# phylo42/RAPPAS

Hardware: AMD Instinct MI355X
Metric: reads placed/sec (whole node), 150 bp DNA vs 10^7-kmer DB (higher is better)
Workload: dtype f32; 1 GPU; C2: DNA k=10, 999 branches, phylo-kmer DB of 786432 keys / 9995042 entries (seed 42), replicated per GPU; 10000000 x 150 symbol reads per GPU per step (uniform, seed 1+rank), keep_at_most=7; reads_per_gpu=10000000

## Files before the change

rappas_amd/csrc/rk_kernels.hip:

```cpp
#include "rk_device.h"
#include "rk_slots24.h"

#include <type_traits>
#ifndef RK_ROW_NT
#define RK_ROW_NT 0
#endif
#ifndef RK_ROW_AUX
#define RK_ROW_AUX 0
#endif
#ifndef RK_HEADS_MAX_K
#define RK_HEADS_MAX_K 16
#endif
#ifndef RK_ABLATE
#define RK_ABLATE 0
#endif
#include "../../include/rappas_place.h"

namespace rk {

#ifdef RK_STAMPS
__device__ unsigned long long rk_stamp_buf[2 * 4096 * 16];
__device__ __forceinline__ unsigned long long rk_now() {
    unsigned long long t;
    __builtin_amdgcn_sched_barrier(0);
    asm volatile("s_memtime %0\n\ts_waitcnt lgkmcnt(0)" : "=s"(t)::"memory");
    __builtin_amdgcn_sched_barrier(0);
    return t;
}
#define RK_STAMP(slot) do { unsigned long long n_ = rk_now(); st_[slot] += n_ - t_; t_ = n_; } while (0)
#define RK_STAMP_PARAMS , unsigned long long *st_, unsigned long long &t_
#define RK_STAMP_ARGS , st_, t_
#else
#define RK_STAMP(slot) do {} while (0)
#define RK_STAMP_PARAMS
#define RK_STAMP_ARGS
#endif

__device__ __forceinline__ u32 ord_f32(float f) {
    u32 u = __float_as_uint(f);
    return (u & 0x80000000u) ? ~u : (u | 0x80000000u);
}
__device__ __forceinline__ float unord_f32(u32 o) {
    u32 u = (o & 0x80000000u) ? (o & 0x7FFFFFFFu) : ~o;
    return __uint_as_float(u);
}
__device__ __forceinline__ u64 make_key(u32 raw_score_bits, u32 branch) {
    return ((u64)ord_f32(__uint_as_float(raw_score_bits)) << 32) | (u64)(0xFFFFu - branch);
}
__device__ __forceinline__ u64 shfl64(u64 v, int src, int width) {
    u32 lo = (u32)v, hi = (u32)(v >> 32);
    lo = __shfl(lo, src, width);
    hi = __shfl(hi, src, width);
    return ((u64)hi << 32) | lo;
}
__device__ __forceinline__ u64 shfl_xor64(u64 v, int m, int width) {
    u32 lo = (u32)v, hi = (u32)(v >> 32);
    lo = __shfl_xor(lo, m, width);
    hi = __shfl_xor(hi, m, width);
    return ((u64)hi << 32) | lo;
}
__device__ __forceinline__ double shfl_f64(double v, int src, int width) {
    return __longlong_as_double((long long)shfl64((u64)__double_as_longlong(v), src, width));
}
__device__ __forceinline__ bool tile_order_given(const PlaceArgs &a) { return a.perm != nullptr && *a.keep_order == 0u; }
__device__ __forceinline__ u32 batch_class(const PlaceArgs &a) { return a.keep_order[0] == 0u ? 2u : (a.keep_order[3] != 0u ? 1u : 0u); }
__device__ __forceinline__ bool batch_is_mine(const PlaceArgs &a) {
    if (!a.only_if || !a.perm) return true;
    return ((a.only_if >> batch_class(a)) & 1u) != 0u;
// ... 203 lines not shown
    c.cur = need ? off : c.cur;
    if (SOA) c.scur = need ? (off_t)(off + 2 * (off_t)len) : c.scur;
    const bool ok = lii < c.rem;
    if (SOA) {
        const off_t bo = ok ? (off_t)(c.cur + 2 * li) : (off_t)0;
        const off_t so = ok ? (off_t)(c.scur + 4 * li) : (off_t)0;
        br = *(const unsigned short *)(rows + bo);
        sc = *(const float *)(rows + so);
        c.cur += 2 * G;
        c.scur += 4 * G;
    } else {
        off_t eo = ok ? (off_t)(c.cur + 8 * li) : (off_t)0;
        if (RK_ABLATE & 16) eo = 0;
        const uint2 e = *(const uint2 *)(rows + eo);
        br = e.x;
        sc = __uint_as_float(e.y);
        c.cur += 8 * G;
    }
    c.rem -= G;
}

__device__ __forceinline__ void apply_entry(u32 *S, u32 nb, u32 br, float sc, float QT, float T, u32 br_base = 0) {
    if (RK_ABLATE & 8) {
        asm volatile("" ::"v"(br), "v"(sc));
        return;
    }
    const u32 idx = (br != 0xFFFFu) ? br - br_base : nb;
    const u32 old = S[idx];
    const float base = (old == S_UNTOUCHED) ? QT : __uint_as_float(old);
    const float d = sc - T;
    const float nw = base + d;
    S[idx] = __float_as_uint(nw);
}
template <bool MONO>
__device__ __forceinline__ float touch_base(u32 old, float QT) {
    float base;
    if (MONO) asm("v_max_f32 %0, %1, %2" : "=v"(base) : "v"(old), "v"(QT));
    else base = (old == S_UNTOUCHED) ? QT : __uint_as_float(old);
    return base;
}
template <bool MONO = false>
__device__ __forceinline__ void apply_delta(u32 *p, float d, float QT) {
    if (RK_ABLATE & 8) {
        asm volatile("" ::"v"(p), "v"(d));
        return;
    }
    *p = __float_as_uint(touch_base<MONO>(*p, QT) + d);
}
template <bool MONO = false>
__device__ __forceinline__ void apply_slot(u32 *S, u32 sb, float sc, float QT, float T) {
    apply_delta<MONO>((u32 *)((unsigned char *)S + sb), sc - T, QT);
}
template <int G, int U, bool WIDE, bool SOA = false>
__device__ __forceinline__ void accumulate_list(u32 *S, u32 nb, const u64 *list, int cnt, u32 li,
                                                const unsigned char *rows, float QT, float T, u32 s_lo = 0, u32 s_win = 0xFFFFu,
                                                u32 wlo4p4 = 4u, u32 w4 = 0xFFFFFFFFu) {
    Cursor<WIDE> c;
    c.h = -1; c.rem = 0; c.cur = 0; c.scur = 0;
    c.dn = list[0];
    u32 br[U];
    float sc[U];
#pragma unroll
    for (int u = 0; u < U; u++) cursor_issue<G, WIDE, SOA>(c, list, cnt, li, (int)li, rows, br[u], sc[u], s_lo, s_win);
    const bool win = !SOA && w4 != 0xFFFFFFFFu;
    auto slot_of = [&](u32 b) {
        if (SOA) {
            const u32 xw = b - s_lo;
            return (xw < s_win) ? (xw + 1u) * 4u : 0u;
        }
        const u32 t = b - wlo4p4;
        return win ? ((t < w4) ? t + 4u : 0u) : b;
    };
    while (true) {
#pragma unroll
        for (int u = 0; u < U; u++) {
            apply_slot(S, slot_of(br[u]), sc[u], QT, T);
            cursor_issue<G, WIDE, SOA>(c, list, cnt, li, (int)li, rows, br[u], sc[u], s_lo, s_win);
        }
        if (!__any(c.h < cnt)) break;
    }
#pragma unroll
    for (int u = 0; u < U; u++) apply_slot(S, slot_of(br[u]), sc[u], QT, T);
}

// ... 29 lines not shown

template <int G, int U, bool WIDE>
__device__ __forceinline__ void accumulate_chunks(u32 *S, u32 nb, const typename ItemT<WIDE>::type *items, int cnt,
                                                  u32 li, const unsigned char *rows, float QT, float T) {
    typedef typename ItemT<WIDE>::type item_t;
    const u32 li8 = li * 8;
    u32 br[U];
    float sc[U];
    item_t it[U];
#pragma unroll
    for (int u = 0; u < U; u++) chunk_issue<G, WIDE>(items[u], u < cnt, li, li8, rows, br[u], sc[u]);
#pragma unroll
    for (int u = 0; u < U; u++) it[u] = items[U + u];
    int s0 = 0;
    while (true) {
#pragma unroll
        for (int u = 0; u < U; u++) {
            apply_slot(S, br[u], sc[u], QT, T);
            chunk_issue<G, WIDE>(it[u], s0 + U + u < cnt, li, li8, rows, br[u], sc[u]);
            it[u] = items[s0 + 2 * U + u];
        }
        s0 += U;
        if (!__any(s0 < cnt)) break;
    }
}

constexpr u32 ITEM_FILLER = 0xFFFFFF00u;
typedef u32 v2u32 __attribute__((ext_vector_type(2)));

__device__ __forceinline__ __amdgpu_buffer_rsrc_t rows_resource(const DbView &db) {
    return __builtin_amdgcn_make_buffer_rsrc((void *)db.rows, (short)0, (int)(u32)db.rows_bytes, 0x00020000);
}

template <int G, int U, bool MONO, bool WIN = false, bool D24 = false>
__device__ __forceinline__ void accumulate_units(u32 *S, const u32 *items, int wcnt, u32 li,
                                                 __amdgpu_buffer_rsrc_t rs, float QT, float T, u32 wlo4p4 = 4u, u32 w4 = 0xFFFFFFFFu) {
    static_assert(!D24 || (G == 16 && !WIN), "dense units: 16-lane groups, whole trees");
    static_assert(rk_slots24::SLOT_BITS == SLOT24_BITS, "rk_slots24.h unpacks the slot words rk_device.h defines");
    const u32 li8 = li * 8;
    const u32 my_unit = li >> 4;
    const rk_slots24::Shifts sh24 = rk_slots24::lane_shifts(li);
    u32 sb[U], it[U];
    float sc[U];
    auto issue = [&](u32 item, u32 &b, float &v) {
        u32 off = item + li8;
        if (G > 16) off = (my_unit <= (item & 7u)) ? (item & ~127u) + li8 : ITEM_FILLER;
        if (RK_ABLATE & 16) off = li8;
        const v2u32 e = __builtin_amdgcn_raw_buffer_load_b64(rs, (int)off, 0, RK_ROW_AUX);
        b = e.x;
        v = __uint_as_float(e.y);
    };
    auto slot_of = [&](u32 b) {
        if (!WIN) return b;
        const u32 t = b - wlo4p4;
        return (t < w4) ? t + 4u : 0u;
    };
    auto prepare = [&](float v, u32 *&pa, u32 *&pb) {
        const int w = (int)__float_as_uint(v);
        const u32 r = (u32)__builtin_amdgcn_update_dpp(w, w, 0x128, 0xF, 0x3, false);
        const rk_slots24::Slots s = rk_slots24::lane_slots(sh24, r);
        pa = S + s.a;
        pb = S + s.b;
    };
#pragma unroll
    for (int u = 0; u < U; u++) issue(items[u], sb[u], sc[u]);
#pragma unroll
    for (int u = 0; u < U; u++) it[u] = items[U + u];
    int s0 = 0;
    if (D24) {
        u32 *pa, *pb;
        prepare(sc[0], pa, pb);
        while (true) {
#pragma unroll
            for (int u = 0; u < U; u++) {
                u32 *na, *nb;
                if (RK_ABLATE & 8) {
                    asm volatile("" ::"v"(pa), "v"(pb), "v"(sb[u]), "v"(sc[u]));
                    prepare(sc[(u + 1) % U], na, nb);
                } else {
                    const u32 oa = *pa, ob = *pb;
                    prepare(sc[(u + 1) % U], na, nb);
                    *pa = __float_as_uint(touch_base<MONO>(oa, QT) + __uint_as_float(sb[u]));
                    *pb = __float_as_uint(touch_base<MONO>(ob, QT) + sc[u]);
                }
                issue(it[u], sb[u], sc[u]);
                it[u] = items[s0 + 2 * U + u];
                pa = na;
                pb = nb;
            }
            s0 += U;
            if (s0 >= wcnt) break;
        }
        return;
    }
    while (true) {
#pragma unroll
        for (int u = 0; u < U; u++) {
            apply_slot<MONO>(S, slot_of(sb[u]), sc[u], QT, T);
            issue(it[u], sb[u], sc[u]);
            it[u] = items[s0 + 2 * U + u];
        }
        s0 += U;
        if (s0 >= wcnt) break;
    }
}

template <int S>
__device__ __forceinline__ u32 row_ror32(u32 v) {
    return (u32)__builtin_amdgcn_update_dpp(0, (int)v, 0x120 + S, 0xF, 0xF, false);
}
template <int G, int S>
__device__ __forceinline__ u64 group_rotate(u64 v, u32 li) {
    if (G == 16) {
        return ((u64)row_ror32<S>((u32)(v >> 32)) << 32) | row_ror32<S>((u32)v);
    } else {
        return shfl64(v, (int)((li + G - S) % G), G);
    }
}
template <int G, int S>
struct RankAbove {
    static __device__ __forceinline__ int run(u64 v, u32 li) {
        return ((group_rotate<G, S>(v, li) > v) ? 1 : 0) + RankAbove<G, S - 1>::run(v, li);
    }
};
template <int G>
struct RankAbove<G, 0> {
    static __device__ __forceinline__ int run(u64, u32) { return 0; }
};
template <int G>
__device__ __forceinline__ u64 group_max(u64 v) {
    if (G == 16) {
        u64 o;
        o = ((u64)row_ror32<8>((u32)(v >> 32)) << 32) | row_ror32<8>((u32)v); v = o > v ? o : v;
        o = ((u64)row_ror32<4>((u32)(v >> 32)) << 32) | row_ror32<4>((u32)v); v = o > v ? o : v;
        o = ((u64)row_ror32<2>((u32)(v >> 32)) << 32) | row_ror32<2>((u32)v); v = o > v ? o : v;
        o = ((u64)row_ror32<1>((u32)(v >> 32)) << 32) | row_ror32<1>((u32)v); v = o > v ? o : v;
        return v;
    } else {
#pragma unroll
        for (int s = 1; s < G; s <<= 1) {
            u64 o = shfl_xor64(v, s, G);
            v = o > v ? o : v;
        }
        return v;
    }
}

template <int G>
__device__ __forceinline__ int rank_candidates(const u64 *list, int c, u64 *win, int K, u32 li) {
    if (c <= G) {
        const u64 mine = ((int)li < c) ? list[li] : 0ull;
        const int rank = RankAbove<G, G - 1>::run(mine, li);
        if (mine != 0 && rank < K) win[rank] = mine;
    } else {
        for (int j = (int)li; j < c; j += G) {
            const u64 mine = list[j];
            int rank = 0;
            for (int t = 0; t < c; t++) rank += (list[t] > mine) ? 1 : 0;
            if (rank < K) win[rank] = mine;
        }
    }
    wave_lds_fence();
    return c < K ? c : K;
}

template <int G>
__device__ __forceinline__ int select_topk_scan(u32 *S, u32 ns, u32 li, u32 gi, int K, u64 *list, int cap, u64 &win_key RK_STAMP_PARAMS) {
    const u32 nb = ns;
    u64 *win = list + (cap - 16);
    const int capc = cap - 16;
    const uint4 *S4 = (const uint4 *)S;
    uint4 *S4w = (uint4 *)S;
    const u32 n4 = (nb + 3) / 4;
    float mo = -INFINITY;
    u32 mi = 0xFFFFFFFFu;
    for (u32 q = li; q < n4; q += G) {
        const uint4 v4 = S4[q];
        const u32 i = 4 * q;
        const float v[4] = {__uint_as_float(v4.x), __uint_as_float(v4.y), __uint_as_float(v4.z), __uint_as_float(v4.w)};
#pragma unroll
        for (int e = 0; e < 4; e++) {
            const bool gt = (v[e] > mo) && (i + e < nb);
            mo = gt ? v[e] : mo;
            mi = gt ? i + e : mi;
        }
    }
    const u64 km = (mi != 0xFFFFFFFFu) ? make_key(__float_as_uint(mo), mi - 1u) : 0ull;
    const int rank = RankAbove<G, G - 1>::run(km, li);
    u64 tau = group_max<G>((rank == K - 1) ? km : 0ull);
    int c = 0;
    const uint4 reset4 = make_uint4(S_UNTOUCHED, S_UNTOUCHED, S_UNTOUCHED, S_UNTOUCHED);
    for (u32 q0 = 0; q0 < n4; q0 += G) {
        const u32 q = q0 + li;
        uint4 v4 = reset4;
        if (q < n4) { v4 = S4[q]; S4w[q] = reset4; }
        const u32 i = 4 * q;
        const u32 raw[4] = {v4.x, v4.y, v4.z, v4.w};
        u64 key[4];
        bool any = false;
#pragma unroll
        for (int e = 0; e < 4; e++) {
            key[e] = (raw[e] != S_UNTOUCHED && i + e < nb) ? make_key(raw[e], i + e - 1u) : 0ull;
            any = any || (key[e] != 0 && key[e] >= tau);
        }
        if (group_bits<G>(__ballot(any), gi) == 0) continue;
#pragma unroll
        for (int e = 0; e < 4; e++) {
            const bool cand = key[e] != 0 && key[e] >= tau;
            const u64 sub = group_bits<G>(__ballot(cand), gi);
            if (sub == 0) continue;
            if (c + G > capc) {
                wave_lds_fence();
                const int kept = rank_candidates<G>(list, c, win, K, li);
                if ((int)li < kept) list[li] = win[li];
                if (kept == K) tau = win[K - 1];
                wave_lds_fence();
                c = kept;
            }
            const bool still = cand && key[e] >= tau;
            const u64 sub2 = group_bits<G>(__ballot(still), gi);
            if (still) list[c + count_below<G>(sub2, li)] = key[e];
            c += __builtin_popcountll(sub2);
        }
    }
    wave_lds_fence();
    const int num = rank_candidates<G>(list, c, win, K, li);
    win_key = ((int)li < num) ? win[li] : 0ull;
// ... 186 lines not shown
    const u32 n4_full = ns / 4;
    if (li < n4_full) {
        uint4 a = S4[li];
        u32 q = li + G;
        for (; q + G < n4_full; q += 2 * G) {
            const uint4 b = S4[q];
            heads3_feed_quad(h, a);
            a = S4[q + G];
            heads3_feed_quad(h, b);
        }
        if (q < n4_full) {
            const uint4 b = S4[q];
            heads3_feed_quad(h, a);
            a = b;
        }
        heads3_feed_quad(h, a);
    }
    if ((ns & 3u) && (n4_full % G) == li) {
        uint4 v4 = S4[n4_full];
        const u32 i = 4 * n4_full;
        if (i >= ns) v4.x = S_UNTOUCHED;
        if (i + 1 >= ns) v4.y = S_UNTOUCHED;
        if (i + 2 >= ns) v4.z = S_UNTOUCHED;
        if (i + 3 >= ns) v4.w = S_UNTOUCHED;
        heads3_feed_quad(h, v4);
    }
}
template <int S>
__device__ __forceinline__ u32 row_shr32(u32 v) {
    return (u32)__builtin_amdgcn_update_dpp(0, (int)v, 0x110 + S, 0xF, 0xF, true);
}
constexpr u32 HEADS3_SECOND = 128u;
template <int G>
__device__ __forceinline__ int heads3_rounds(const Heads3 &h, int K, u32 li, u32 gi, u32 &win_o, u32 &win_t, bool &doubt) {
    static_assert(4 * G < (int)HEADS3_SECOND, "stream tags");
    constexpr u32 ORD_NEG_INF = 0x007FFFFFu;
    u32 o0[4], o1[4], t0[4];
#pragma unroll
    for (int c = 0; c < 4; c++) {
        o0[c] = ord_f32(h.s0[c]); o1[c] = ord_f32(h.s1[c]);
        t0[c] = 4u * li + (u32)c + 1u;
    }
    u32 last = ORD_NEG_INF;
    int num = 0;
    win_o = 0; win_t = 0;
    for (int r = 0; r < K; r++) {
        const u32 m = group_max_u32<G>(max(max(o0[0], o0[1]), max(o0[2], o0[3])));
        const bool valid = m != ORD_NEG_INF;
        u32 cand = 0;
#pragma unroll
        for (int c = 0; c < 4; c++) cand = max(cand, (o0[c] == m) ? t0[c] : 0u);
        const u32 w = group_max_u32<G>(valid ? cand : 0u);
        const bool mine = (int)li == r && valid;
        win_o = mine ? m : win_o;
        win_t = mine ? w : win_t;
        num += valid ? 1 : 0;
        last = valid ? m : last;
#pragma unroll
        for (int c = 0; c < 4; c++) {
            const bool pop = valid && t0[c] == w;
            o0[c] = pop ? o1[c] : o0[c];
            o1[c] = pop ? ORD_NEG_INF : o1[c];
            t0[c] = pop ? (t0[c] | HEADS3_SECOND) : t0[c];
        }
    }
    u32 od = max(max(ord_f32(h.dr[0]), ord_f32(h.dr[1])), max(ord_f32(h.dr[2]), ord_f32(h.dr[3])));
    od = max(od, max(max(o0[0], o0[1]), max(o0[2], o0[3])));
    const bool d = (num == K) ? (od >= last) : (od != ORD_NEG_INF);
    doubt = group_bits<G>(__ballot(d), gi) != 0;
    return num;
}
template <int G>
__device__ __forceinline__ u32 heads3_locate(const u32 *S, u32 ns, u32 stream, u32 bits, bool second) {
    constexpr u32 NONE = 0x40000000u;
    constexpr int CH = 8;
    const u32 n4 = (ns + 3) / 4;
    const int trip = (int)((n4 + G - 1) / G);
    const int cnt = (int)((ns - stream + 4u * G - 1u) / (4u * G));
    int k = (trip - 1) / CH;
    const u32 *p = S + stream + (u32)(4 * G * CH) * (u32)k;
    u32 first = NONE, sec = NONE;
    {
        const int jv = cnt - CH * k;
        u32 w[CH];
#pragma unroll
        for (int j = 0; j < CH; j++) {
            const u32 *pj = (j < jv) ? p + 4 * G * j : S;
            w[j] = *pj;
        }
#pragma unroll
        for (int j = CH - 1; j >= 0; j--) {
            const bool eq = w[j] == bits;
            sec = eq ? first : sec;
            first = eq ? (u32)j : first;
        }
    }
    for (k--; k >= 0; k--) {
        p -= 4 * G * CH;
        first += (u32)CH; sec += (u32)CH;
        u32 w[CH];
#pragma unroll
        for (int j = 0; j < CH; j++) w[j] = p[4 * G * j];
#pragma unroll
        for (int j = CH - 1; j >= 0; j--) {
            const bool eq = w[j] == bits;
            sec = eq ? first : sec;
            first = eq ? (u32)j : first;
        }
    }
    const u32 i = second ? sec : first;
    return i < NONE ? stream + 4u * G * i : 0u;
}
template <int G>
__device__ __forceinline__ int heads3_select(u32 *S, u32 ns, u32 li, u32 gi, int K, u64 *list, int cap, u64 &win_key, bool &doubt RK_STAMP_PARAMS) {
    Heads3 h;
    heads3_clear(h);
    heads3_scan<G>(S, ns, li, h);
    RK_STAMP(8);
    u32 win_o, win_t;
    const int num = heads3_rounds<G>(h, K, li, gi, win_o, win_t, doubt);
    RK_STAMP(9);
    const bool won = (int)li < num;
    const u32 prev_o = row_shr32<1>(win_o), prev_t = row_shr32<1>(win_t);
    const bool tie = won && li > 0 && prev_o == win_o;
    const bool second = tie && (prev_t | HEADS3_SECOND) == win_t;
    const u32 stream = won ? (win_t & (HEADS3_SECOND - 1u)) - 1u : 0u;
    const u32 slot = heads3_locate<G>(S, ns, stream, __float_as_uint(unord_f32(win_o)), second);
    if (group_bits<G>(__ballot(won && slot == 0u), gi) != 0) doubt = true;
    win_key = won ? (((u64)win_o << 32) | (u64)(0xFFFFu - (slot - 1u))) : 0ull;
    if (__ballot(tie && !doubt) != 0) {
#ifdef RK_STAMPS
        st_[15] += 1;
#endif
        wave_lds_fence();
        if (won) list[li] = win_key;
        wave_lds_fence();
        u64 *win = list + (cap - 16);
        rank_candidates<G>(list, num, win, K, li);
        win_key = won ? win[li] : 0ull;
        wave_lds_fence();
    }
    RK_STAMP(13);
    return num;
}
template <int G>
__device__ __forceinline__ int select_topk(u32 *S, u32 n_branches, u32 li, u32 gi, int K, u64 *list, int cap, u64 &win_key RK_STAMP_PARAMS) {
    if (li == 0) S[0] = S_UNTOUCHED;
    wave_lds_fence();
    const u32 nb = n_branches + 1;
    if (K > RK_HEADS_MAX_K || K > G) return select_topk_scan<G>(S, nb, li, gi, K, list, cap, win_key RK_STAMP_ARGS);
    bool doubt;
    int num;
    if constexpr (G == 16) {
        num = heads3_select<G>(S, nb, li, gi, K, list, cap, win_key, doubt RK_STAMP_ARGS);
    } else {
        Heads4 h;
        heads_clear(h);
        heads_scan<G>(S, nb, li, 0u, h);
        RK_STAMP(8);
        num = heads_rounds<G>(h, K, li, gi, win_key, doubt);
    }
#ifdef RK_STAMPS
    st_[14] += doubt ? 1 : 0;
#endif
    if (doubt) return select_topk_scan<G>(S, nb, li, gi, K, list, cap, win_key RK_STAMP_ARGS);
    RK_STAMP(9);
    uint4 *S4w = (uint4 *)S;
    const u32 n4 = (nb + 3) / 4;
    const uint4 reset4 = make_uint4(S_UNTOUCHED, S_UNTOUCHED, S_UNTOUCHED, S_UNTOUCHED);
    for (u32 q = li; q < n4; q += G) S4w[q] = reset4;
    return num;
}

template <int G>
__device__ __forceinline__ void heads_scan_reset(u32 *S, u32 n_branches, u32 li, u32 slot_base, Heads4 &h) {
    if (li == 0) S[0] = S_UNTOUCHED;
    wave_lds_fence();
    heads_scan<G, true>(S, n_branches + 1, li, slot_base, h);
}

template <int LANE>
__device__ __forceinline__ u32 row_bcast32(u32 v) {
    return (u32)__builtin_amdgcn_update_dpp(0, (int)v, 0x150 + LANE, 0xF, 0xF, false);
}

template <int G>
__device__ __forceinline__ void weigh_and_store(const PlaceArgs &a, u64 r, u32 li, int numBest, u64 win_key,
                                                u32 flags) {
    const int K = (int)a.keep_at_most;
    float score = unord_f32((u32)(win_key >> 32));
    u32 branch = 0xFFFFu - (u32)(win_key & 0xFFFFu);
    int n_rows = 0;
    double lwr = 0.0;
    if (numBest > 0 && !(RK_ABLATE & 4)) {
        flags |= RK_FLAG_PLACED;
        const bool mine = (int)li < numBest;
        float best, lowest;
        if (G == 16) {
            best = __uint_as_float(row_bcast32<0>(__float_as_uint(score)));
            float lo = mine ? score : INFINITY;
            lo = fminf(lo, __uint_as_float(row_ror32<8>(__float_as_uint(lo))));
            lo = fminf(lo, __uint_as_float(row_ror32<4>(__float_as_uint(lo))));
            lo = fminf(lo, __uint_as_float(row_ror32<2>(__float_as_uint(lo))));
            lowest = fminf(lo, __uint_as_float(row_ror32<1>(__float_as_uint(lo))));
// ... 312 lines not shown
            const u32 mask = (k >= 16) ? 0xFFFFFFFFu : ((1u << (2 * k)) - 1u);
#pragma unroll
            for (int u = 0; u < PU; u++) code[u] = __builtin_amdgcn_alignbit(w[u + 1], w[u], 2 * li) & mask;
            return;
        }
    }
#pragma unroll
    for (int u = 0; u < PU; u++) {
        const u32 j0 = pos + u * 16 + li;
        const u32 j = j0 < Q ? j0 : 0u;
        const u32 bit = j * BITS, wi = bit >> 5, sh = bit & 31;
        const u32 w0 = __shfl(recw, (int)(wi & 15u), 16);
        u32 w1 = __shfl(recw, (int)((wi + 1) & 15u), 16);
        w1 = wi + 1 < 16 ? w1 : 0u;
        const u32 nbits = k * BITS;
        if (nbits <= 32) {
            const u32 c32 = __builtin_amdgcn_alignbit(w1, w0, sh);
            code[u] = nbits == 32 ? c32 : (c32 & ((1u << nbits) - 1u));
            continue;
        }
        u32 w2 = 0u;
        if (BITS * 12 + 31 > 64) {
            w2 = __shfl(recw, (int)((wi + 2) & 15u), 16);
            w2 = (wi + 2 < 16 && nbits + sh > 64) ? w2 : 0u;
        }
        const u64 c = funnel96(w0, w1, w2, sh);
        code[u] = nbits >= 64 ? c : (c & ((1ull << nbits) - 1));
    }
}

template <int BITS, int TM, int U, int PU, bool D24 = false>
__global__ void __launch_bounds__(256) place_packed16_kernel(PlaceArgs a) {
    constexpr int G = 16, NG = 4;
    static_assert(TM != TM_HASH, "direct tables only");
    static_assert(!D24 || TM == TM_COMPACT, "the dense view carries a compact table");
    if (!batch_is_mine(a)) return;
    extern __shared__ u32 lds[];
    const bool perm_given = tile_order_given(a);
    const u32 lane = threadIdx.x & 63;
    const u32 wave = threadIdx.x >> 6;
    const u32 waves_per_block = blockDim.x >> 6;
    const u32 gi = lane / G, li = lane % G;
    const u32 wave_words = NG * (a.s_stride + 2 * a.list_cap);
    u32 *wbase = lds + wave * wave_words;
    u32 *S = wbase + gi * a.s_stride;
    u64 *list = (u64 *)(wbase + NG * a.s_stride) + gi * a.list_cap;
    u32 *items = (u32 *)list;
    const u32 nb = a.db.n_branches;
    const u32 k = a.db.k;
    const float T = a.db.T;
    const __amdgpu_buffer_rsrc_t rows_rs = rows_resource(a.db);
    const int cap_items = (int)(a.list_cap * 2) - 3 * U - 2;
    const int cap_rows = (int)a.list_cap - 1;
    const u32 wpr = a.words_per_read;

    for (u32 i = li; i < a.s_stride; i += G) S[i] = S_UNTOUCHED;
    wave_lds_fence();

    const u64 n_tiles = (a.n_reads + NG - 1) / NG;
    const u64 wave_global = (u64)blockIdx.x * waves_per_block + wave;
    const u64 wave_count = (u64)gridDim.x * waves_per_block;

    auto load_tile = [&](u64 tile, u32 &recw, u32 &R, u32 &fin, bool &have) {
        const u64 slot = tile * NG + gi;
        have = tile < n_tiles && slot < a.n_reads;
        const u64 r = have ? tile_read(a, slot, perm_given) : 0ull;
        recw = 0; R = 0; fin = 0;
        if (have) {
            if (li < wpr) recw = a.packed[r * wpr + li];
            R = a.lens ? a.lens[r] : a.fixed_len;
            fin = a.flags_in ? a.flags_in[r] : 0u;
        }
    };
    auto mer_count = [&](u32 R, u32 fin, bool have) -> u32 {
        const u32 cap_syms = (wpr * 32u) / BITS;
        R = R < cap_syms ? R : cap_syms;
        const bool is_amb = (fin & RK_FLAG_AMBIGUOUS) != 0;
        const bool rejected = (fin & (RK_FLAG_BAD_CHAR | RK_FLAG_TOO_LONG)) != 0;
        return (have && !is_amb && !rejected && R >= k) ? (R - k + 1) : 0u;
    };
    auto fetch_batch = [&](u32 recw, u32 pos, u32 Q, u64 (&code)[PU], RawSlot (&raw)[PU]) {
        record_codes<BITS, PU>(recw, pos, li, k, Q, code);
#pragma unroll
        for (int u = 0; u < PU; u++) raw[u] = lookup_fetch<BITS, TM>(a.db, code[u]);
    };
    auto decode_batch = [&](const u64 (&code)[PU], const RawSlot (&raw)[PU], u32 pos, u32 Q, u64 (&desc)[PU]) {
#pragma unroll
        for (int u = 0; u < PU; u++) {
            const u32 j = pos + u * G + li;
            const u64 d = lookup_decode<BITS, TM>(a.db, raw[u], code[u]);
            desc[u] = j < Q ? d : 0ull;
        }
    };

#ifdef RK_STAMPS
    unsigned long long st_[16] = {0, 0, 0, 0, 0, 0, 0, 0, 0, 0, 0, 0, 0, 0, 0, 0};
    unsigned long long t_ = rk_now();
#endif
    u32 c_recw, c_R, c_fin;
    bool c_have;
    u64 desc0[PU];
    {
        load_tile(wave_global, c_recw, c_R, c_fin, c_have);
        u64 code[PU];
        RawSlot raw[PU];
        const u32 Q0 = mer_count(c_R, c_fin, c_have);
        fetch_batch(c_recw, 0u, Q0, code, raw);
        decode_batch(code, raw, 0u, Q0, desc0);
    }

    for (u64 tile = wave_global; tile < n_tiles; tile += wave_count) {
        const bool have = c_have;
        const u64 r = have ? tile_read(a, tile * NG + gi, perm_given) : 0ull;
        const u32 fin = c_fin;
        u32 R = c_R;
        {
            const u32 cap_syms = (wpr * 32u) / BITS;
            R = R < cap_syms ? R : cap_syms;
        }
        u32 flags = fin & (RK_FLAG_BAD_CHAR | RK_FLAG_AMBIGUOUS | RK_FLAG_TOO_LONG);
        const bool is_amb = (fin & RK_FLAG_AMBIGUOUS) != 0;
        const bool rejected = (fin & (RK_FLAG_BAD_CHAR | RK_FLAG_TOO_LONG)) != 0;
        if (R < k) flags |= RK_FLAG_TOO_SHORT;
        const u32 Q = mer_count(c_R, fin, have);
        const float QT = (float)(int)Q * T;

        int cnt = 0;
        auto flush = [&]() {
            int wcnt = __builtin_amdgcn_readlane(cnt, 0);
            wcnt = max(wcnt, __builtin_amdgcn_readlane(cnt, 32));
            wcnt = max(wcnt, __builtin_amdgcn_readlane(cnt, 16));
            wcnt = max(wcnt, __builtin_amdgcn_readlane(cnt, 48));
            for (int i = cnt + (int)li; i < wcnt + 2 * U; i += G) items[i] = ITEM_FILLER;
            wave_lds_fence();
            if (a.db.mono) accumulate_units<G, U, true, false, D24>(S, items, wcnt, li, rows_rs, QT, T);
            else accumulate_units<G, U, false, false, D24>(S, items, wcnt, li, rows_rs, QT, T);
            wave_lds_fence();
            cnt = 0;
        };
        auto emit_batch = [&](const u64 (&desc)[PU], bool more) {
            u32 nch[PU], excl[PU];
            int total = 0;
            bool wide_rows = false;
#pragma unroll
            for (int u = 0; u < PU; u++) {
                const u32 lenp = (u32)desc[u] & DESC_LEN_MASK;
                nch[u] = (lenp + G - 1) >> 4;
                wide_rows = wide_rows || nch[u] > 15u;
            }
            auto row_scan = [](u32 v) {
                v += (u32)__builtin_amdgcn_update_dpp(0, (int)v, 0x111, 0xF, 0xF, true);
                v += (u32)__builtin_amdgcn_update_dpp(0, (int)v, 0x112, 0xF, 0xF, true);
                v += (u32)__builtin_amdgcn_update_dpp(0, (int)v, 0x114, 0xF, 0xF, true);
                v += (u32)__builtin_amdgcn_update_dpp(0, (int)v, 0x118, 0xF, 0xF, true);
                return v;
            };
            if (!__any(wide_rows)) {
#pragma unroll
                for (int u0 = 0; u0 < PU; u0 += 4) {
                    u32 packed = nch[u0];
                    if (u0 + 1 < PU) packed |= nch[u0 + 1 < PU ? u0 + 1 : u0] << 8;
                    if (u0 + 2 < PU) packed |= nch[u0 + 2 < PU ? u0 + 2 : u0] << 16;
                    if (u0 + 3 < PU) packed |= nch[u0 + 3 < PU ? u0 + 3 : u0] << 24;
                    const u32 incl = row_scan(packed);
                    const u32 tot = row_bcast32<15>(incl);
#pragma unroll
                    for (int b = 0; b < 4; b++) {
                        if (u0 + b < PU) {
                            const int u = u0 + b < PU ? u0 + b : u0;
                            excl[u] = (u32)total + ((incl >> (8 * b)) & 0xFFu) - nch[u];
                            total += (int)((tot >> (8 * b)) & 0xFFu);
                        }
                    }
                }
            } else {
#pragma unroll
                for (int u = 0; u < PU; u++) {
                    const u32 incl = row_scan(nch[u]);
                    excl[u] = (u32)total + incl - nch[u];
                    total += (int)row_bcast32<15>(incl);
                }
            }
            if (__any(more && cnt + total > cap_items)) flush();
            if (D24 && __any(more && total > cap_items)) {
                for (u32 done = 0; __any(done < (u32)total);) {
                    const u32 room = (u32)(cap_items - cnt);
#pragma unroll
                    for (int u = 0; u < PU; u++) {
                        const u32 rb = (u32)(desc[u] >> DESC_LEN_BITS) * 8u;
                        for (u32 c = 0; __any(c < nch[u]); c++) {
                            const u32 x = excl[u] + c - done;
                            if (c < nch[u] && x < room) items[cnt + (int)x] = rb + c * 128u;
                        }
                    }
                    const u32 take = min((u32)total - done, room);
                    cnt += (int)take;
                    done += take;
                    if (__any(done < (u32)total)) flush();
                }
            } else if (__any(more && total > cap_items)) {
                const int per_part = cap_rows / G;
                for (int u_lo = 0; u_lo < PU; u_lo += per_part) {
                    int rc = 0;
#pragma unroll
                    for (int u = 0; u < PU; u++) {
                        const bool part = u >= u_lo && u < u_lo + per_part;
                        const bool hit = part && ((u32)desc[u] & DESC_LEN_MASK) != 0;
                        const u64 bal = __ballot(hit);
                        const u64 sub = group_bits<G>(bal, gi);
                        if (hit) list[rc + count_below<G>(sub, li)] = desc[u];
                        rc += __builtin_popcountll(sub);
                    }
                    if (li == 0) list[rc] = 0;
                    wave_lds_fence();
                    if (__any(rc > 0)) accumulate_list<G, U, false>(S, nb, list, rc, li, a.db.rows, QT, T);
                    wave_lds_fence();
                }
            } else {
#pragma unroll
                for (int u = 0; u < PU; u++) {
                    const u32 rb = (u32)(desc[u] >> DESC_LEN_BITS) * 8u;
                    const int base = cnt + (int)excl[u];
                    if (nch[u] > 0) items[base] = rb;
                    if (nch[u] > 1) items[base + 1] = rb + 128u;
                    for (u32 c = 2; __any(c < nch[u]); c++)
                        if (c < nch[u]) items[base + (int)c] = rb + c * 128u;
                }
                cnt += total;
            }
        };

        RK_STAMP(0);
        emit_batch(desc0, Q > 0);
        for (u32 pos = PU * G; __any(pos < Q); pos += PU * G) {
            u64 code[PU], desc[PU];
            RawSlot raw[PU];
            fetch_batch(c_recw, pos, Q, code, raw);
            __builtin_amdgcn_sched_barrier(0);
            decode_batch(code, raw, pos, Q, desc);
            emit_batch(desc, pos < Q);
        }
        RK_STAMP(2);
        load_tile(tile + wave_count, c_recw, c_R, c_fin, c_have);
        if (__any(cnt > 0)) flush();
        RK_STAMP(4);
        u64 ncode[PU];
        RawSlot nraw[PU];
        const u32 nQ = mer_count(c_R, c_fin, c_have);
        fetch_batch(c_recw, 0u, nQ, ncode, nraw);
        __builtin_amdgcn_sched_barrier(0);
        RK_STAMP(1);

        u64 win_key;
        int numBest = 0;
        if (RK_ABLATE & 2) { win_key = list[0]; for (u32 i = li; i <= nb; i += G) S[i] = S_UNTOUCHED; }
        else numBest = select_topk<G>(S, nb, li, gi, (int)a.keep_at_most, list, (int)a.list_cap, win_key RK_STAMP_ARGS);
        wave_lds_fence();
        RK_STAMP(5);
        decode_batch(ncode, nraw, 0u, nQ, desc0);
        __builtin_amdgcn_sched_barrier(0);
        RK_STAMP(3);
        const bool deferred = is_amb && a.has_ascii && !rejected;
        if (have && !deferred) weigh_and_store<G>(a, r, li, numBest, win_key, flags);
        RK_STAMP(6);
    }
#ifdef RK_STAMPS
    if (lane == 0 && wave_global < 4096)
        for (int i = 0; i < 16; i++) rk_stamp_buf[wave_global * 16 + i] = st_[i];
#endif
}

constexpr int RETILE_BINS = 64;
template <int BITS>
__device__ __forceinline__ u32 retile_read_key(const PlaceArgs &a, u64 r, u32 &spread, u32 *with_row = nullptr) {
    const u32 k = a.db.k, wpr = a.words_per_read;
    u32 R = a.lens ? a.lens[r] : a.fixed_len;
    const u32 cap_syms = (wpr * 32u) / BITS;
    R = R < cap_syms ? R : cap_syms;
    const u32 fin = a.flags_in ? a.flags_in[r] : 0u;
    const bool plain = (fin & (RK_FLAG_BAD_CHAR | RK_FLAG_AMBIGUOUS | RK_FLAG_TOO_LONG)) == 0 && R >= k;
    u32 key = 0;
    spread = 0;
    if (plain) {
        const u32 Q = R - k + 1;
        const u32 *rec = a.packed + r * wpr;
        constexpr int NS = 7;
        u32 w[NS];
#pragma unroll
        for (int i = 0; i < NS; i++) {
            const u32 p_ = (u32)(((u64)(Q - 1) * (u32)i) / (NS - 1));
            w[i] = a.db.winspec[(u32)dense_index<BITS>(extract_code<BITS>(rec, wpr, p_, k), k)] & 63u;
        }
        u32 best = 0, best_n = 0;
#pragma unroll
// ... 2204 lines not shown
```

Baseline: 412.0 million reads/s.

## Prime accumulate row loads early and trim padded tail iterations

Adds an EDGE mode to accumulate_units. When the first batch fits, the first NP unit row loads are issued during emit_batch, before decoding the remaining k-mers, and carried into the flush in a UnitRing so their latency overlaps the decode. The main loop also stops at the last full U-group and finishes the remainder in a bounded tail loop, so filler slots are no longer processed. This adds register pressure for the held ring values and more code paths. Correctness relies on the ring being invalidated whenever an early flush happens.

```diff
diff --git a/rappas_amd/csrc/rk_kernels.hip b/rappas_amd/csrc/rk_kernels.hip
--- a/rappas_amd/csrc/rk_kernels.hip
+++ b/rappas_amd/csrc/rk_kernels.hip
@@ -30,10 +30,18 @@
 #define RK_STAMP(slot) do { unsigned long long n_ = rk_now(); st_[slot] += n_ - t_; t_ = n_; } while (0)
 #define RK_STAMP_PARAMS , unsigned long long *st_, unsigned long long &t_
 #define RK_STAMP_ARGS , st_, t_
+#define RK_ACC_STAMP_PARAMS , unsigned long long *acc_st_ = nullptr
+#define RK_ACC_STAMP_ARGS , st_
+#define RK_ACC_STAMP_BEGIN unsigned long long acc_t0_ = acc_st_ ? rk_now() : 0ull
+#define RK_ACC_STAMP_FIRST do { if (acc_st_ && acc_t0_) { acc_st_[7] += rk_now() - acc_t0_; acc_t0_ = 0ull; } } while (0)
 #else
 #define RK_STAMP(slot) do {} while (0)
 #define RK_STAMP_PARAMS
 #define RK_STAMP_ARGS
+#define RK_ACC_STAMP_PARAMS
+#define RK_ACC_STAMP_ARGS
+#define RK_ACC_STAMP_BEGIN do {} while (0)
+#define RK_ACC_STAMP_FIRST do {} while (0)
 #endif
 
 __device__ __forceinline__ u32 ord_f32(float f) {
@@ -416,24 +424,33 @@
     return __builtin_amdgcn_make_buffer_rsrc((void *)db.rows, (short)0, (int)(u32)db.rows_bytes, 0x00020000);
 }
 
-template <int G, int U, bool MONO, bool WIN = false, bool D24 = false>
+template <int NP>
+struct UnitRing {
+    u32 sb[NP];
+    float sc[NP];
+    bool primed;
+};
+template <int G>
+__device__ __forceinline__ void unit_issue(__amdgpu_buffer_rsrc_t rs, u32 item, u32 li, u32 &b, float &v) {
+    const u32 li8 = li * 8;
+    u32 off = item + li8;
+    if (G > 16) off = ((li >> 4) <= (item & 7u)) ? (item & ~127u) + li8 : ITEM_FILLER;
+    if (RK_ABLATE & 16) off = li8;
+    const v2u32 e = __builtin_amdgcn_raw_buffer_load_b64(rs, (int)off, 0, RK_ROW_AUX);
+    b = e.x;
+    v = __uint_as_float(e.y);
+}
+
+template <int G, int U, bool MONO, bool WIN = false, bool D24 = false, bool EDGE = false, int NP = U>
 __device__ __forceinline__ void accumulate_units(u32 *S, const u32 *items, int wcnt, u32 li,
-                                                 __amdgpu_buffer_rsrc_t rs, float QT, float T, u32 wlo4p4 = 4u, u32 w4 = 0xFFFFFFFFu) {
+                                                 __amdgpu_buffer_rsrc_t rs, float QT, float T, u32 wlo4p4 = 4u, u32 w4 = 0xFFFFFFFFu,
+                                                 const UnitRing<NP> *pre = nullptr RK_ACC_STAMP_PARAMS) {
     static_assert(!D24 || (G == 16 && !WIN), "dense units: 16-lane groups, whole trees");
     static_assert(rk_slots24::SLOT_BITS == SLOT24_BITS, "rk_slots24.h unpacks the slot words rk_device.h defines");
-    const u32 li8 = li * 8;
-    const u32 my_unit = li >> 4;
     const rk_slots24::Shifts sh24 = rk_slots24::lane_shifts(li);
     u32 sb[U], it[U];
     float sc[U];
-    auto issue = [&](u32 item, u32 &b, float &v) {
-        u32 off = item + li8;
-        if (G > 16) off = (my_unit <= (item & 7u)) ? (item & ~127u) + li8 : ITEM_FILLER;
-        if (RK_ABLATE & 16) off = li8;
-        const v2u32 e = __builtin_amdgcn_raw_buffer_load_b64(rs, (int)off, 0, RK_ROW_AUX);
-        b = e.x;
-        v = __uint_as_float(e.y);
-    };
+    auto issue = [&](u32 item, u32 &b, float &v) { unit_issue<G>(rs, item, li, b, v); };
     auto slot_of = [&](u32 b) {
         if (!WIN) return b;
         const u32 t = b - wlo4p4;
@@ -446,8 +463,16 @@
         pa = S + s.a;
         pb = S + s.b;
     };
-#pragma unroll
-    for (int u = 0; u < U; u++) issue(items[u], sb[u], sc[u]);
+    RK_ACC_STAMP_BEGIN;
+    if (EDGE && pre->primed) {
+#pragma unroll
+        for (int u = 0; u < NP; u++) { sb[u] = pre->sb[u]; sc[u] = pre->sc[u]; }
+#pragma unroll
+        for (int u = NP; u < U; u++) issue(items[u], sb[u], sc[u]);
+    } else {
+#pragma unroll
+        for (int u = 0; u < U; u++) issue(items[u], sb[u], sc[u]);
+    }
 #pragma unroll
     for (int u = 0; u < U; u++) it[u] = items[U + u];
     int s0 = 0;
@@ -455,6 +480,7 @@
         u32 *pa, *pb;
         prepare(sc[0], pa, pb);
         while (true) {
+            if (EDGE && s0 + U > wcnt) break;
 #pragma unroll
             for (int u = 0; u < U; u++) {
                 u32 *na, *nb;
@@ -471,13 +497,35 @@
                 it[u] = items[s0 + 2 * U + u];
                 pa = na;
                 pb = nb;
+                if (u == 0) RK_ACC_STAMP_FIRST;
             }
             s0 += U;
-            if (s0 >= wcnt) break;
+            if (!EDGE && s0 >= wcnt) break;
+        }
+        if (EDGE) {
+            const int rem = wcnt - s0;
+#pragma unroll
+            for (int u = 0; u < U - 1; u++) {
+                if (u >= rem) break;
+                u32 *na, *nb;
+                if (RK_ABLATE & 8) {
+                    asm volatile("" ::"v"(pa), "v"(pb), "v"(sb[u]), "v"(sc[u]));
+                    prepare(sc[u + 1], na, nb);
+                } else {
+                    const u32 oa = *pa, ob = *pb;
+                    prepare(sc[u + 1], na, nb);
+                    *pa = __float_as_uint(touch_base<MONO>(oa, QT) + __uint_as_float(sb[u]));
+                    *pb = __float_as_uint(touch_base<MONO>(ob, QT) + sc[u]);
+                }
+                pa = na;
+                pb = nb;
+                if (u == 0) RK_ACC_STAMP_FIRST;
+            }
         }
         return;
     }
     while (true) {
+        if (EDGE && s0 + U > wcnt) break;
 #pragma unroll
         for (int u = 0; u < U; u++) {
             apply_slot<MONO>(S, slot_of(sb[u]), sc[u], QT, T);
@@ -485,7 +533,15 @@
             it[u] = items[s0 + 2 * U + u];
         }
         s0 += U;
-        if (s0 >= wcnt) break;
+        if (!EDGE && s0 >= wcnt) break;
+    }
+    if (EDGE) {
+        const int rem = wcnt - s0;
+#pragma unroll
+        for (int u = 0; u < U - 1; u++) {
+            if (u >= rem) break;
+            apply_slot<MONO>(S, slot_of(sb[u]), sc[u], QT, T);
+        }
     }
 }
 
@@ -1345,6 +1401,8 @@
 template <int BITS, int TM, int U, int PU, bool D24 = false>
 __global__ void __launch_bounds__(256) place_packed16_kernel(PlaceArgs a) {
     constexpr int G = 16, NG = 4;
+    constexpr bool EDGE = !(RK_ABLATE & 16384);
+    constexpr int NP = BITS == 5 ? U / 2 : U;
     static_assert(TM != TM_HASH, "direct tables only");
     static_assert(!D24 || TM == TM_COMPACT, "the dense view carries a compact table");
     if (!batch_is_mine(a)) return;
@@ -1439,19 +1497,27 @@
         const float QT = (float)(int)Q * T;
 
         int cnt = 0;
-        auto flush = [&]() {
-            int wcnt = __builtin_amdgcn_readlane(cnt, 0);
-            wcnt = max(wcnt, __builtin_amdgcn_readlane(cnt, 32));
-            wcnt = max(wcnt, __builtin_amdgcn_readlane(cnt, 16));
-            wcnt = max(wcnt, __builtin_amdgcn_readlane(cnt, 48));
+        UnitRing<NP> ring;
+        ring.primed = false;
+        auto flush = [&]() __attribute__((always_inline)) {
+            const int c0 = __builtin_amdgcn_readlane(cnt, 0), c1 = __builtin_amdgcn_readlane(cnt, 16);
+            const int c2 = __builtin_amdgcn_readlane(cnt, 32), c3 = __builtin_amdgcn_readlane(cnt, 48);
+            const int wcnt = max(max(c0, c2), max(c1, c3));
+#ifdef RK_STAMPS
+            st_[10] += (unsigned long long)(EDGE ? 0 : (wcnt + U - 1) / U * U + (wcnt ? 0 : U) - wcnt);
+            st_[11] += (unsigned long long)(4 * wcnt - c0 - c1 - c2 - c3);
+            st_[12] += 1ull;
+#endif
             for (int i = cnt + (int)li; i < wcnt + 2 * U; i += G) items[i] = ITEM_FILLER;
             wave_lds_fence();
-            if (a.db.mono) accumulate_units<G, U, true, false, D24>(S, items, wcnt, li, rows_rs, QT, T);
-            else accumulate_units<G, U, false, false, D24>(S, items, wcnt, li, rows_rs, QT, T);
+            if (a.db.mono) accumulate_units<G, U, true, false, D24, EDGE, NP>(S, items, wcnt, li, rows_rs, QT, T, 4u, 0xFFFFFFFFu, &ring RK_ACC_STAMP_ARGS);
+            else accumulate_units<G, U, false, false, D24, EDGE, NP>(S, items, wcnt, li, rows_rs, QT, T, 4u, 0xFFFFFFFFu, &ring RK_ACC_STAMP_ARGS);
             wave_lds_fence();
             cnt = 0;
+            ring.primed = false;
         };
-        auto emit_batch = [&](const u64 (&desc)[PU], bool more) {
+        auto emit_batch = [&](const u64 (&desc)[PU], bool more, auto first) {
+            constexpr bool FIRST = EDGE && decltype(first)::value;
             u32 nch[PU], excl[PU];
             int total = 0;
             bool wide_rows = false;
@@ -1468,6 +1534,14 @@
                 v += (u32)__builtin_amdgcn_update_dpp(0, (int)v, 0x118, 0xF, 0xF, true);
                 return v;
             };
+            auto write_items = [&](int u, int at) {
+                const u32 rb = (u32)(desc[u] >> DESC_LEN_BITS) * 8u;
+                const int base = at + (int)excl[u];
+                if (nch[u] > 0) items[base] = rb;
+                if (nch[u] > 1) items[base + 1] = rb + 128u;
+                for (u32 c = 2; __any(c < nch[u]); c++)
+                    if (c < nch[u]) items[base + (int)c] = rb + c * 128u;
+            };
             if (!__any(wide_rows)) {
 #pragma unroll
                 for (int u0 = 0; u0 < PU; u0 += 4) {
@@ -1485,6 +1559,16 @@
                             total += (int)((tot >> (8 * b)) & 0xFFu);
                         }
                     }
+                    if (FIRST && u0 == 0) {
+                        const u32 tot0 = tot & 0xFFu;
+                        if (__any(more) && !__any(more && (tot0 < (u32)NP || tot0 > (u32)cap_items))) {
+                            write_items(0, 0);
+                            wave_lds_fence();
+#pragma unroll
+                            for (int t = 0; t < NP; t++) unit_issue<G>(rows_rs, more ? items[t] : ITEM_FILLER, li, ring.sb[t], ring.sc[t]);
+                            ring.primed = true;
+                        }
+                    }
                 }
             } else {
 #pragma unroll
@@ -1494,7 +1578,10 @@
                     total += (int)row_bcast32<15>(incl);
                 }
             }
-            if (__any(more && cnt + total > cap_items)) flush();
+            if (__any(more && cnt + total > cap_items)) {
+                if (FIRST) ring.primed = false;
+                flush();
+            }
             if (D24 && __any(more && total > cap_items)) {
                 for (u32 done = 0; __any(done < (u32)total);) {
                     const u32 room = (u32)(cap_items - cnt);
@@ -1531,27 +1618,21 @@
                 }
             } else {
 #pragma unroll
-                for (int u = 0; u < PU; u++) {
-                    const u32 rb = (u32)(desc[u] >> DESC_LEN_BITS) * 8u;
-                    const int base = cnt + (int)excl[u];
-                    if (nch[u] > 0) items[base] = rb;
-                    if (nch[u] > 1) items[base + 1] = rb + 128u;
-                    for (u32 c = 2; __any(c < nch[u]); c++)
-                        if (c < nch[u]) items[base + (int)c] = rb + c * 128u;
-                }
+                for (int u = 0; u < PU; u++)
+                    if (!(FIRST && u == 0 && ring.primed)) write_items(u, cnt);
                 cnt += total;
             }
         };
 
         RK_STAMP(0);
-        emit_batch(desc0, Q > 0);
+        emit_batch(desc0, Q > 0, std::true_type());
         for (u32 pos = PU * G; __any(pos < Q); pos += PU * G) {
             u64 code[PU], desc[PU];
             RawSlot raw[PU];
             fetch_batch(c_recw, pos, Q, code, raw);
             __builtin_amdgcn_sched_barrier(0);
             decode_batch(code, raw, pos, Q, desc);
-            emit_batch(desc, pos < Q);
+            emit_batch(desc, pos < Q, std::false_type());
         }
         RK_STAMP(2);
         load_tile(tile + wave_count, c_recw, c_R, c_fin, c_have);
```

Measured after the change: 412.8 million reads/s, median of 5. About the same (+0.2%).

## Pre-seed score slots with Q*threshold to drop per-touch untouched checks

Applied to the files above, without the earlier changes.

Instead of resetting the per-branch score array to an 'untouched' sentinel, the kernel seeds every slot with Q*T for the next read. Accumulation then becomes a plain load-add-store without the max or compare against the threshold. Top-k selection uses the heads3 fast path with a tau floor. When the seeded result cannot be proven equal to the original semantics, the read is recomputed with sentinel-initialised scores. This adds a rare redo path and changes how resets are written.

```diff
diff --git a/rappas_amd/csrc/rk_kernels.hip b/rappas_amd/csrc/rk_kernels.hip
--- a/rappas_amd/csrc/rk_kernels.hip
+++ b/rappas_amd/csrc/rk_kernels.hip
@@ -303,24 +303,25 @@
     const float nw = base + d;
     S[idx] = __float_as_uint(nw);
 }
-template <bool MONO>
+template <bool MONO, bool SEEDED = false>
 __device__ __forceinline__ float touch_base(u32 old, float QT) {
     float base;
-    if (MONO) asm("v_max_f32 %0, %1, %2" : "=v"(base) : "v"(old), "v"(QT));
+    if (SEEDED) base = __uint_as_float(old);
+    else if (MONO) asm("v_max_f32 %0, %1, %2" : "=v"(base) : "v"(old), "v"(QT));
     else base = (old == S_UNTOUCHED) ? QT : __uint_as_float(old);
     return base;
 }
-template <bool MONO = false>
+template <bool MONO = false, bool SEEDED = false>
 __device__ __forceinline__ void apply_delta(u32 *p, float d, float QT) {
     if (RK_ABLATE & 8) {
         asm volatile("" ::"v"(p), "v"(d));
         return;
     }
-    *p = __float_as_uint(touch_base<MONO>(*p, QT) + d);
-}
-template <bool MONO = false>
+    *p = __float_as_uint(touch_base<MONO, SEEDED>(*p, QT) + d);
+}
+template <bool MONO = false, bool SEEDED = false>
 __device__ __forceinline__ void apply_slot(u32 *S, u32 sb, float sc, float QT, float T) {
-    apply_delta<MONO>((u32 *)((unsigned char *)S + sb), sc - T, QT);
+    apply_delta<MONO, SEEDED>((u32 *)((unsigned char *)S + sb), sc - T, QT);
 }
 template <int G, int U, bool WIDE, bool SOA = false>
 __device__ __forceinline__ void accumulate_list(u32 *S, u32 nb, const u64 *list, int cnt, u32 li,
@@ -416,7 +417,7 @@
     return __builtin_amdgcn_make_buffer_rsrc((void *)db.rows, (short)0, (int)(u32)db.rows_bytes, 0x00020000);
 }
 
-template <int G, int U, bool MONO, bool WIN = false, bool D24 = false>
+template <int G, int U, bool MONO, bool WIN = false, bool D24 = false, bool SEEDED = false>
 __device__ __forceinline__ void accumulate_units(u32 *S, const u32 *items, int wcnt, u32 li,
                                                  __amdgpu_buffer_rsrc_t rs, float QT, float T, u32 wlo4p4 = 4u, u32 w4 = 0xFFFFFFFFu) {
     static_assert(!D24 || (G == 16 && !WIN), "dense units: 16-lane groups, whole trees");
@@ -464,8 +465,8 @@
                 } else {
                     const u32 oa = *pa, ob = *pb;
                     prepare(sc[(u + 1) % U], na, nb);
-                    *pa = __float_as_uint(touch_base<MONO>(oa, QT) + __uint_as_float(sb[u]));
-                    *pb = __float_as_uint(touch_base<MONO>(ob, QT) + sc[u]);
+                    *pa = __float_as_uint(touch_base<MONO, SEEDED>(oa, QT) + __uint_as_float(sb[u]));
+                    *pb = __float_as_uint(touch_base<MONO, SEEDED>(ob, QT) + sc[u]);
                 }
                 issue(it[u], sb[u], sc[u]);
                 it[u] = items[s0 + 2 * U + u];
@@ -480,7 +481,7 @@
     while (true) {
 #pragma unroll
         for (int u = 0; u < U; u++) {
-            apply_slot<MONO>(S, slot_of(sb[u]), sc[u], QT, T);
+            apply_slot<MONO, SEEDED>(S, slot_of(sb[u]), sc[u], QT, T);
             issue(it[u], sb[u], sc[u]);
             it[u] = items[s0 + 2 * U + u];
         }
@@ -549,7 +550,8 @@
 }
 
 template <int G>
-__device__ __forceinline__ int select_topk_scan(u32 *S, u32 ns, u32 li, u32 gi, int K, u64 *list, int cap, u64 &win_key RK_STAMP_PARAMS) {
+__device__ __forceinline__ int select_topk_scan(u32 *S, u32 ns, u32 li, u32 gi, int K, u64 *list, int cap, u64 &win_key RK_STAMP_PARAMS,
+                                                u32 reset_word = S_UNTOUCHED, u64 tau_floor = 0ull) {
     const u32 nb = ns;
     u64 *win = list + (cap - 16);
     const int capc = cap - 16;
@@ -572,11 +574,12 @@
     const u64 km = (mi != 0xFFFFFFFFu) ? make_key(__float_as_uint(mo), mi - 1u) : 0ull;
     const int rank = RankAbove<G, G - 1>::run(km, li);
     u64 tau = group_max<G>((rank == K - 1) ? km : 0ull);
+    tau = tau > tau_floor ? tau : tau_floor;
     int c = 0;
-    const uint4 reset4 = make_uint4(S_UNTOUCHED, S_UNTOUCHED, S_UNTOUCHED, S_UNTOUCHED);
+    const uint4 reset4 = make_uint4(reset_word, reset_word, reset_word, reset_word);
     for (u32 q0 = 0; q0 < n4; q0 += G) {
         const u32 q = q0 + li;
-        uint4 v4 = reset4;
+        uint4 v4 = make_uint4(S_UNTOUCHED, S_UNTOUCHED, S_UNTOUCHED, S_UNTOUCHED);
         if (q < n4) { v4 = S4[q]; S4w[q] = reset4; }
         const u32 i = 4 * q;
         const u32 raw[4] = {v4.x, v4.y, v4.z, v4.w};
@@ -829,7 +832,7 @@
 }
 constexpr u32 HEADS3_SECOND = 128u;
 template <int G>
-__device__ __forceinline__ int heads3_rounds(const Heads3 &h, int K, u32 li, u32 gi, u32 &win_o, u32 &win_t, bool &doubt) {
+__device__ __forceinline__ int heads3_rounds(const Heads3 &h, int K, u32 li, u32 gi, u32 &win_o, u32 &win_t, bool &doubt, u32 *kth_o = nullptr) {
     static_assert(4 * G < (int)HEADS3_SECOND, "stream tags");
     constexpr u32 ORD_NEG_INF = 0x007FFFFFu;
     u32 o0[4], o1[4], t0[4];
@@ -865,6 +868,7 @@
     od = max(od, max(max(o0[0], o0[1]), max(o0[2], o0[3])));
     const bool d = (num == K) ? (od >= last) : (od != ORD_NEG_INF);
     doubt = group_bits<G>(__ballot(d), gi) != 0;
+    if (kth_o) *kth_o = (num == K) ? last : ORD_NEG_INF;
     return num;
 }
 template <int G>
@@ -909,13 +913,14 @@
     return i < NONE ? stream + 4u * G * i : 0u;
 }
 template <int G>
-__device__ __forceinline__ int heads3_select(u32 *S, u32 ns, u32 li, u32 gi, int K, u64 *list, int cap, u64 &win_key, bool &doubt RK_STAMP_PARAMS) {
+__device__ __forceinline__ int heads3_select(u32 *S, u32 ns, u32 li, u32 gi, int K, u64 *list, int cap, u64 &win_key, bool &doubt RK_STAMP_PARAMS,
+                                             u32 *kth_o = nullptr) {
     Heads3 h;
     heads3_clear(h);
     heads3_scan<G>(S, ns, li, h);
     RK_STAMP(8);
     u32 win_o, win_t;
-    const int num = heads3_rounds<G>(h, K, li, gi, win_o, win_t, doubt);
+    const int num = heads3_rounds<G>(h, K, li, gi, win_o, win_t, doubt, kth_o);
     RK_STAMP(9);
     const bool won = (int)li < num;
     const u32 prev_o = row_shr32<1>(win_o), prev_t = row_shr32<1>(win_t);
@@ -967,6 +972,44 @@
     const uint4 reset4 = make_uint4(S_UNTOUCHED, S_UNTOUCHED, S_UNTOUCHED, S_UNTOUCHED);
     for (u32 q = li; q < n4; q += G) S4w[q] = reset4;
     return num;
+}
+
+template <int G>
+__device__ __forceinline__ int select_topk_seeded(u32 *S, u32 n_branches, u32 li, u32 gi, int K, u64 *list, int cap, u64 &win_key,
+                                                  bool seeded, float QT, bool work, u32 next_seed, bool &redo RK_STAMP_PARAMS) {
+    static_assert(G == 16, "the fast select of 16-lane groups");
+    if (li == 0) S[0] = S_UNTOUCHED;
+    wave_lds_fence();
+    const u32 nb = n_branches + 1;
+    const u32 qt_o = ord_f32(QT);
+    bool doubt = false;
+    int num = 0;
+    u32 kth_o = 0;
+    win_key = 0ull;
+    const bool fast = K <= RK_HEADS_MAX_K && K <= G;
+    if (fast) num = heads3_select<G>(S, nb, li, gi, K, list, cap, win_key, doubt RK_STAMP_ARGS, &kth_o);
+    redo = seeded && work && !(fast && num == K && kth_o > qt_o);
+    if (!seeded) doubt = doubt || !fast;
+    else if (!work || redo) doubt = false;
+#ifdef RK_STAMPS
+    st_[14] += doubt ? 1 : 0;
+    st_[12] += redo ? 1 : 0;
+#endif
+    if (seeded && !work) { num = 0; win_key = 0ull; }
+    if (doubt) return select_topk_scan<G>(S, nb, li, gi, K, list, cap, win_key RK_STAMP_ARGS, next_seed, seeded ? ((u64)qt_o + 1ull) << 32 : 0ull);
+    RK_STAMP(9);
+    uint4 *S4w = (uint4 *)S;
+    const u32 n4 = (nb + 3) / 4;
+    const uint4 reset4 = make_uint4(next_seed, next_seed, next_seed, next_seed);
+    for (u32 q = li; q < n4; q += G) S4w[q] = reset4;
+    return num;
+}
+template <int G>
+__device__ __forceinline__ void fill_scores(u32 *S, u32 n_branches, u32 li, u32 word) {
+    uint4 *S4w = (uint4 *)S;
+    const u32 n4 = (n_branches + 1 + 3) / 4;
+    const uint4 w4 = make_uint4(word, word, word, word);
+    for (u32 q = li; q < n4; q += G) S4w[q] = w4;
 }
 
 template <int G>
@@ -1366,9 +1409,8 @@
     const int cap_items = (int)(a.list_cap * 2) - 3 * U - 2;
     const int cap_rows = (int)a.list_cap - 1;
     const u32 wpr = a.words_per_read;
-
-    for (u32 i = li; i < a.s_stride; i += G) S[i] = S_UNTOUCHED;
-    wave_lds_fence();
+    const bool seeded = a.db.mono != 0u;
+    auto seed_of = [&](u32 Qn) -> u32 { return seeded ? __float_as_uint((float)(int)Qn * T) : S_UNTOUCHED; };
 
     const u64 n_tiles = (a.n_reads + NG - 1) / NG;
     const u64 wave_global = (u64)blockIdx.x * waves_per_block + wave;
@@ -1419,6 +1461,9 @@
         RawSlot raw[PU];
         const u32 Q0 = mer_count(c_R, c_fin, c_have);
         fetch_batch(c_recw, 0u, Q0, code, raw);
+        const u32 seed0 = seed_of(Q0);
+        for (u32 i = li; i < a.s_stride; i += G) S[i] = seed0;
+        wave_lds_fence();
         decode_batch(code, raw, 0u, Q0, desc0);
     }
 
@@ -1439,6 +1484,8 @@
         const float QT = (float)(int)Q * T;
 
         int cnt = 0;
+        bool had_units = false;
+        bool marker = false;
         auto flush = [&]() {
             int wcnt = __builtin_amdgcn_readlane(cnt, 0);
             wcnt = max(wcnt, __builtin_amdgcn_readlane(cnt, 32));
@@ -1446,7 +1493,7 @@
             wcnt = max(wcnt, __builtin_amdgcn_readlane(cnt, 48));
             for (int i = cnt + (int)li; i < wcnt + 2 * U; i += G) items[i] = ITEM_FILLER;
             wave_lds_fence();
-            if (a.db.mono) accumulate_units<G, U, true, false, D24>(S, items, wcnt, li, rows_rs, QT, T);
+            if (seeded && !marker) accumulate_units<G, U, true, false, D24, true>(S, items, wcnt, li, rows_rs, QT, T);
             else accumulate_units<G, U, false, false, D24>(S, items, wcnt, li, rows_rs, QT, T);
             wave_lds_fence();
             cnt = 0;
@@ -1494,6 +1541,7 @@
                     total += (int)row_bcast32<15>(incl);
                 }
             }
+            had_units = had_units || total > 0;
             if (__any(more && cnt + total > cap_items)) flush();
             if (D24 && __any(more && total > cap_items)) {
                 for (u32 done = 0; __any(done < (u32)total);) {
@@ -1566,13 +1614,40 @@
 
         u64 win_key;
         int numBest = 0;
-        if (RK_ABLATE & 2) { win_key = list[0]; for (u32 i = li; i <= nb; i += G) S[i] = S_UNTOUCHED; }
-        else numBest = select_topk<G>(S, nb, li, gi, (int)a.keep_at_most, list, (int)a.list_cap, win_key RK_STAMP_ARGS);
+        bool redo = false;
+        const u32 next_seed = seed_of(nQ);
+        if (RK_ABLATE & 2) { win_key = list[0]; for (u32 i = li; i <= nb; i += G) S[i] = next_seed; }
+        else numBest = select_topk_seeded<G>(S, nb, li, gi, (int)a.keep_at_most, list, (int)a.list_cap, win_key, seeded, QT, Q > 0 && had_units, next_seed, redo RK_STAMP_ARGS);
         wave_lds_fence();
         RK_STAMP(5);
         decode_batch(ncode, nraw, 0u, nQ, desc0);
         __builtin_amdgcn_sched_barrier(0);
         RK_STAMP(3);
+        if (__builtin_expect(__any(redo), 0)) {
+            u32 recw2 = 0;
+            if (redo && li < wpr) recw2 = a.packed[r * wpr + li];
+            const u32 Q2 = redo ? Q : 0u;
+            fill_scores<G>(S, nb, li, S_UNTOUCHED);
+            wave_lds_fence();
+            marker = true;
+            for (u32 pos = 0; __any(pos < Q2); pos += PU * G) {
+                u64 code[PU], desc[PU];
+                RawSlot raw[PU];
+                fetch_batch(recw2, pos, Q2, code, raw);
+                __builtin_amdgcn_sched_barrier(0);
+                decode_batch(code, raw, pos, Q2, desc);
+                emit_batch(desc, pos < Q2);
+            }
+            if (__any(cnt > 0)) flush();
+            marker = false;
+            u64 key2;
+            const int num2 = select_topk<G>(S, nb, li, gi, (int)a.keep_at_most, list, (int)a.list_cap, key2 RK_STAMP_ARGS);
+            wave_lds_fence();
+            if (redo) { numBest = num2; win_key = key2; }
+            fill_scores<G>(S, nb, li, next_seed);
+            wave_lds_fence();
+            RK_STAMP(7);
+        }
         const bool deferred = is_amb && a.has_ascii && !rejected;
         if (have && !deferred) weigh_and_store<G>(a, r, li, numBest, win_key, flags);
         RK_STAMP(6);
```

After: 411.8 million reads/s before, 363.4 million reads/s after. 11.8% lower.
